# cv-stuttgart/PCFA

Hardware: AMD Instinct MI355X
Metric: attack_steps_per_sec (higher is better)
Workload: dtype f32; 1 GPU; RAFT, 1 synthetic 436x1024 pair per GPU (padded 440x1024), disjoint delta, change_of_variables, delta_bound=0.005, zero target, L-BFGS max_iter=10; weights=random:1234, parallelism=pairs sharded 1/GPU, closure_launch=hipGraph replay

## Files before the change

include/pcfa_hip.h:

```cpp
#ifndef PCFA_HIP_H
#define PCFA_HIP_H

#include <stddef.h>
#include <stdint.h>

#ifdef __cplusplus
extern "C" {
#endif

#define PCFA_OK 0
#define PCFA_ERR_INVALID_ARG (-1)
#define PCFA_ERR_UNSUPPORTED (-2)
#define PCFA_ERR_WORKSPACE (-3)

#if defined(__GNUC__)
#define PCFA_API __attribute__((visibility("default")))
#else
#define PCFA_API
#endif

#define PCFA_MAX_LEVELS 8
#define PCFA_ABI_VERSION 2

#define PCFA_LOSS_AEE 0
// ... 221 lines not shown
PCFA_API int pcfa_leaky_relu_fwd(const float* x, float* y, float slope, long long n, void* stream);
PCFA_API int pcfa_leaky_relu_bwd(const float* out, const float* grad_out, float* grad_x, float slope, long long n,
                        void* stream);
PCFA_API int pcfa_conv3x3_act_fwd_pair(const float* x, const float* packed, const float* bias, float* out, int K, int N,
                              const float* x2, const float* packed2, const float* bias2, float* out2, int K2, int N2,
                              int H, int W, int act, float slope, void* stream);
PCFA_API int pcfa_conv3x3_fused_bwd(const float* g, const float* packed_bwd, const float* mask, const float* addend,
                           float* grad_in, int B, int K, int N, int H, int W, void* stream);
PCFA_API int pcfa_conv3x3_masked_fwd(const float* x, const float* packed, const float* mask, float* out, int B, int K,
                            int N, int H, int W, void* stream);
PCFA_API int pcfa_conv3x3_algo(int B, int K, int N, int H, int W);
PCFA_API size_t pcfa_conv3x3_workspace_bytes(int B, int K, int N, int H, int W);
PCFA_API int pcfa_conv3x3_run(const float* x, const float* packed, const float* bias, const float* mask,
                     const float* addend, float* out, int B, int K, int N, int H, int W, int act, float slope,
                     int mask_channels, void* workspace, size_t workspace_bytes, void* stream);

PCFA_API int pcfa_bias_relu_fwd(const float* x, const float* bias, float* out, long long n, int plane, int channels,
                       void* stream);
PCFA_API int pcfa_relu_bwd(const float* out, const float* grad_out, float* grad_x, long long n, void* stream);
PCFA_API int pcfa_relu_bwd2(const float* out, const float* out2, const float* grad_out, float* grad_x, float* grad_x2,
                   long long n, void* stream);

PCFA_API int pcfa_conv_fewin_fwd(const float* x, const float* w, const float* bias, float* out, int B, int Cin, int N,
                                 int H, int W, int ksize, int relu, void* stream);
PCFA_API long long pcfa_conv_fewin_packed_floats(int Cin, int N, int ksize);
PCFA_API int pcfa_conv_fewin_pack(const float* w, float* packed, int Cin, int N, int ksize, void* stream);
PCFA_API int pcfa_conv_fewin_packed_fwd(const float* x, const float* packed, const float* bias, float* out, int B, int Cin,
                               int N, int H, int W, int ksize, int relu, void* stream);

PCFA_API int pcfa_conv_s2_supported(int Cin, int N, int ksize, int H, int W);
// ... 115 lines not shown
```

pcfa_amd/_hip.py:

```python
import ctypes
import os
from ctypes import c_char_p, c_double, c_float, c_int, c_longlong, c_size_t, c_uint, c_void_p, POINTER

ABI_VERSION = 2
LIB_PATH = os.environ.get("PCFA_HIP_LIB") or os.path.join(os.path.dirname(os.path.abspath(__file__)), "lib",
                                                          "libpcfa_hip.so")

PCFA_LOSS = {"aee": 0, "mse": 1, "cosim": 2}


class HipLibraryError(RuntimeError):
    pass


_P = c_void_p
_S4 = POINTER(c_longlong)

SIGNATURES = {
    "pcfa_abi_version": (c_int, []),
    "pcfa_timing_arm": (c_int, [_P, _P, c_int]),
    "pcfa_null_launch": (c_int, [_P]),
    "pcfa_poison_lds": (c_int, [c_uint, _P]),
    "pcfa_peek_lds": (c_int, [_P, c_int, _P]),
    "pcfa_calib_mfma_f32": (c_longlong, [_P, c_int, c_int, _P]),
# ... 83 lines not shown
                                            c_int, c_int, _P]),
    "pcfa_sepconv5_gru_update_bwd": (c_int, [_P, c_int, c_int, _P, _P, _P, _P, _P, _P, _P, _P, _P, c_int, c_int, c_int,
                                             c_int, _P]),
    "pcfa_convex_upsample_fwd": (c_int, [_P, _P, _P, c_int, c_int, c_int, _P]),
    "pcfa_convex_upsample_workspace_floats": (c_longlong, [c_int, c_int, c_int]),
    "pcfa_convex_upsample_bwd": (c_int, [_P, _P, _P, _P, _P, _P, c_int, c_int, c_int, _P]),
    "pcfa_flow_step": (c_int, [_P, _P, _P, _P, _P, c_longlong, _P]),
    "pcfa_conv3x3_act_fwd_pair": (c_int, [_P, _P, _P, _P, c_int, c_int, _P, _P, _P, _P, c_int, c_int, c_int, c_int, c_int,
                                          c_float, _P]),
    "pcfa_relu_bwd2": (c_int, [_P, _P, _P, _P, _P, c_longlong, _P]),
    "pcfa_conv3x3_fused_bwd": (c_int, [_P, _P, _P, _P, _P, c_int, c_int, c_int, c_int, c_int, _P]),
    "pcfa_conv3x3_masked_fwd": (c_int, [_P, _P, _P, _P, c_int, c_int, c_int, c_int, c_int, _P]),
    "pcfa_conv3x3_algo": (c_int, [c_int] * 5),
    "pcfa_conv3x3_workspace_bytes": (c_size_t, [c_int] * 5),
    "pcfa_conv3x3_run": (c_int, [_P] * 6 + [c_int] * 6 + [c_float, c_int, _P, c_size_t, _P]),
    "pcfa_conv3x3_packed_floats": (c_longlong, [c_int, c_int]),
    "pcfa_conv3x3_pack_weights": (c_int, [_P, _P, _P, c_int, c_int, _P]),
    "pcfa_conv3x3_fwd": (c_int, [_P, _P, _P, _P, c_int, c_int, c_int, c_int, c_int, c_int, _P]),
    "pcfa_conv3x3_act_fwd": (c_int, [_P, _P, _P, _P, c_int, c_int, c_int, c_int, c_int, c_int, c_float, _P]),
    "pcfa_leaky_relu_fwd": (c_int, [_P, _P, c_float, c_longlong, _P]),
    "pcfa_leaky_relu_bwd": (c_int, [_P, _P, _P, c_float, c_longlong, _P]),
    "pcfa_lbfgs_gram_state_bytes": (c_size_t, [c_int]),
    "pcfa_lbfgs_gram_workspace_bytes": (c_size_t, [c_int, c_longlong]),
    "pcfa_lbfgs_gram_reset": (c_int, [_P, c_int, _P]),
    "pcfa_lbfgs_gram_update": (c_int, [_P, _P, _P, c_float, _P, _P, _P, _P, c_int, c_longlong, _P]),
    "pcfa_lbfgs_gram_direction": (c_int, [_P, _P, _P, _P, _P, _P, _P, c_int, c_longlong, _P]),
    "pcfa_lbfgs_workspace_floats": (c_size_t, []),
    "pcfa_lbfgs_pair": (c_int, [_P, _P, _P, c_float, _P, _P, _P, _P, c_int, c_longlong, _P]),
    "pcfa_lbfgs_direction": (c_int, [_P, _P, _P, _P, _P, _P, _P, _P, c_int, c_int, c_int, c_longlong, c_longlong,
                                     _P]),
# ... 96 lines not shown
```

pcfa_amd/config.py:

```python
import dataclasses
import os


def _env_bool(name, default):
    v = os.environ.get(name)
    return default if v is None else v not in ("0", "", "false", "False")


@dataclasses.dataclass(frozen=True)
class Config:
    fused_lookup: bool = True
    overlap_encoders: bool = False
    conv_s2: bool = True
    conv_s2_bwd: bool = True
    fused_downsample: bool = True
    defer_relu: bool = True
    pyramid_bwd_windows: bool = True
    gma_gemm: str = "lib"
    gma_attention: str = "materialised"
    conv1x1: str = "lib"
    corr: str = "all_pairs"
    ondemand_lookup: str = "per_query"
    mfma: str = "f32"
    dilated_as_subgrids: tuple = (2, 4, 8, 16)
    deconv_fewout: bool = True
    defer_leaky: bool = True
    dense_block_fused_masks: bool = True
    warp_bwd_deterministic: bool = True
    pwc_fold_glue: bool = True
    spynet_ops: str = "lib"
    flownet2_ops: str = "lib"
    reuse_pair_graphs: bool = True
    max_cached_shapes: int = 4

    @classmethod
    def from_env(cls):
        return cls(fused_lookup=_env_bool("PCFA_FUSED_LOOKUP", True),
                   overlap_encoders=_env_bool("PCFA_OVERLAP_ENCODERS", False),
                   defer_relu=_env_bool("PCFA_DEFER_RELU", True),
                   gma_gemm=os.environ.get("PCFA_GMA_GEMM", "lib"),
                   gma_attention=os.environ.get("PCFA_GMA_ATTENTION", "materialised"),
                   conv1x1=os.environ.get("PCFA_CONV1X1", "lib"),
                   corr=os.environ.get("PCFA_CORR", "all_pairs"),
                   ondemand_lookup=os.environ.get("PCFA_ONDEMAND_LOOKUP", "per_query"),
                   mfma=os.environ.get("PCFA_MFMA", "f32"),
                   spynet_ops=os.environ.get("PCFA_SPYNET_OPS", "lib"),
                   flownet2_ops=os.environ.get("PCFA_FLOWNET2_OPS", "lib"),
                   max_cached_shapes=int(os.environ.get("PCFA_MAX_CACHED_SHAPES", "4")))

    def __post_init__(self):
        if self.gma_gemm not in ("lib", "hip"):
            raise ValueError("Config.gma_gemm must be 'lib' or 'hip', got %r" % (self.gma_gemm,))
        if self.gma_attention not in ("materialised", "streamed"):
            raise ValueError("Config.gma_attention must be 'materialised' or 'streamed', got %r" % (self.gma_attention,))
        if self.conv1x1 not in ("lib", "hip"):
            raise ValueError("Config.conv1x1 must be 'lib' or 'hip', got %r" % (self.conv1x1,))
        if self.corr not in ("all_pairs", "on_demand"):
            raise ValueError("Config.corr must be 'all_pairs' or 'on_demand', got %r" % (self.corr,))
        if self.ondemand_lookup not in ("per_query", "tiled"):
            raise ValueError("Config.ondemand_lookup must be 'per_query' or 'tiled', got %r" % (self.ondemand_lookup,))
        if self.mfma not in ("f32", "bf16x3"):
            raise ValueError("Config.mfma must be 'f32' or 'bf16x3', got %r" % (self.mfma,))
        if self.spynet_ops not in ("lib", "hip"):
# ... 22 lines not shown
```

pcfa_amd/csrc/conv3x3.hip:

```cpp
#include "common.hpp"
#include "conv3x3_f43.hpp"
#include "conv_tail.hpp"
#include <cstdlib>

namespace {

typedef float f32x16 __attribute__((ext_vector_type(16)));

constexpr int TC = 8;
constexpr int PC = 2 * TC + 2;
constexpr int PCP = 20;
constexpr int KC = 8;
constexpr int CB = 64;

__global__ void conv3x3_pack_kernel(const float* __restrict__ w, float* __restrict__ P, int Cout, int Cin,
                                    int backward, int K, int N, int nchunk, long long total) {
  for (long long e = (long long)blockIdx.x * blockDim.x + threadIdx.x; e < total;
       e += (long long)gridDim.x * blockDim.x) {
    const int pos = (int)(e & 15), lane = (int)((e >> 4) & 63), wv = (int)((e >> 10) & 3);
    const long long blk = e >> 12;
    const int c = (int)(blk % nchunk), nb = (int)(blk / nchunk);
    const int a = pos >> 2, kpi = pos & 3;
    const int i = wv, j = a;
    const int k = 8 * c + 2 * kpi + (lane >> 5), n = 32 * nb + (lane & 31);
// ... 33 lines not shown
  } while (0)
#else
#define C3_STAMP(k) do {} while (0)
#endif

struct Second {
  const float* x;
  const float* U;
  const float* bias;
  float* out;
  int K, N, nb0;
  int mask_n;
  int ksl;
  int cper;
  PcfaXcdMap xcd;
};

template <int ACT, int CBT, int MT, bool KFULL, int NRING, int KS = 1>
__global__ __launch_bounds__(256 * MT * KS) __attribute__((amdgpu_waves_per_eu(KS == 2 ? 2 : (MT == 1 && NRING == 2 && CBT == 32 ? 3 : (CBT == 64 ? 1 : 2))))) void conv3x3_winograd_kernel(
    const float* __restrict__ x, const float* __restrict__ U, const float* __restrict__ bias,
    const float* __restrict__ mask, const float* __restrict__ addend, float* __restrict__ out, int K, int N, int Npad,
    int H, int W, int blocks_x, float slope, Second second) {
  constexpr int NT = 256 * MT;
  constexpr int TR = 4 * MT, TB = TR * TC;
  constexpr int PR = 2 * TR + 2;
  constexpr int RAW = KC * PR * PCP;
  constexpr int RAW_LOADS = (KC * PR * PC + NT - 1) / NT;
  constexpr int MS = TB + 1;
  constexpr int NB = CBT / 32;
  static_assert(KS == 1 || (KS == 2 && MT == 1 && CBT == 32), "split-K rides on the 256-thread tile");
  constexpr int EPI = 16 * 16 * (TB + 1);
  constexpr int RED = KS == 2 ? 4 * 4 * 16 * 64 : 0;
  constexpr int LDS0 = 2 * KS * RAW > EPI ? 2 * KS * RAW : EPI;
  constexpr int LDSF = RED > LDS0 ? RED : LDS0;
  __shared__ __attribute__((aligned(16))) float smem[LDSF];
  const int kgrp = KS == 1 ? 0 : (int)(threadIdx.x >> 8);
  float* sRaw = smem + kgrp * 2 * RAW;

  const int tid = KS == 1 ? (int)threadIdx.x : (int)(threadIdx.x & 255);
  const int lane = tid & 63, wave = (tid >> 6) & 3, mt = tid >> 8;
  const int l31 = lane & 31, lh = lane >> 5;
  int tileblk = blockIdx.x, nby = blockIdx.y;
  if (second.xcd.a != 0 && !pcfa_xcd_item(second.xcd, (int)blockIdx.x, tileblk, nby)) return;
  const int by = tileblk / blocks_x, bx = tileblk - by * blocks_x;
  const int y0 = by * (2 * TR), x0 = bx * (2 * TC);
  if (nby >= second.nb0) {
    nby -= second.nb0;
    x = second.x;
    U = second.U;
    bias = second.bias;
    out = second.out;
    K = second.K;
    N = second.N;
    mask = nullptr;
    addend = nullptr;
  }
  const int mask_n = second.mask_n;
  const int n0 = nby * CBT;
  if (n0 >= N) return;
  const long long plane = (long long)H * W;
  const int ksl = second.ksl, img = blockIdx.z / ksl, slice = blockIdx.z - img * ksl;
  x += (long long)img * K * plane;
  out += ((long long)slice * (gridDim.z / ksl) + img) * N * plane;
  if (mask != nullptr) mask += (long long)img * N * plane;
  if (addend != nullptr) addend += (long long)img * N * plane;

  unsigned praw[RAW_LOADS];
  int rdst[RAW_LOADS];
  int rch[RAW_LOADS];
  bool rok[RAW_LOADS];
#pragma unroll
  for (int i = 0; i < RAW_LOADS; ++i) {
    const int e = tid + NT * i;
    const int ch = e / (PR * PC), rem = e - ch * (PR * PC);
    const int r = rem / PC, c = rem - r * PC;
    const int yy = y0 - 1 + r, xx = x0 - 1 + c;
// ... 201 lines not shown
#pragma unroll
      for (int xi = 0; xi < 16; ++xi) m[xi] = sM[(xi * 16 + cl) * MS + e_tile];
      float t0[4], t1[4];
#pragma unroll
      for (int j = 0; j < 4; ++j) {
        t0[j] = m[j] + m[4 + j] + m[8 + j];
        t1[j] = m[4 + j] - m[8 + j] - m[12 + j];
      }
      const float bv = (bias != nullptr && n < N) ? bias[n] : 0.f;
      const float y00 = t0[0] + t0[1] + t0[2] + bv, y01 = t0[1] - t0[2] - t0[3] + bv;
      const float y10 = t1[0] + t1[1] + t1[2] + bv, y11 = t1[1] - t1[2] - t1[3] + bv;
      if (n < N && oy < H && ox < W && worker) {
        const long long oo = (long long)n * plane + (long long)oy * W + ox;
        const bool mall = mask != nullptr && mask_n == 0, mpre = mask != nullptr && mask_n > 0 && n < mask_n;
        const bool add = addend != nullptr;
        const float4 y = conv_tail<ACT>(make_float4(y00, y01, y10, y11), slope, mall, mpre,
                                        [&] { return make_float4(mk[q][0], mk[q][1], mk[q][2], mk[q][3]); }, add,
                                        [&] { return make_float4(ad[q][0], ad[q][1], ad[q][2], ad[q][3]); });
        float* o = out + oo;
        o[0] = y.x;
        if (ox + 1 < W) o[1] = y.y;
        if (oy + 1 < H) {
          o[W] = y.z;
          if (ox + 1 < W) o[W + 1] = y.w;
        }
      }
    }
    __syncthreads();
  }
}

}

// ... 52 lines not shown
  pcfa_launch(leaky_relu_fwd_kernel, dim3((unsigned)min((n + 255) / 256, 4096LL)), dim3(256), 0, (hipStream_t)stream, x, y,
              slope, n);
  PCFA_LAUNCH_CHECK();
  return PCFA_OK;
}

extern "C" int pcfa_leaky_relu_bwd(const float* out, const float* grad_out, float* grad_x, float slope, long long n,
                                   void* stream) {
  if (!out || !grad_out || !grad_x || n < 1) return PCFA_ERR_INVALID_ARG;
  pcfa_launch(leaky_relu_bwd_kernel, dim3((unsigned)min((n + 255) / 256, 4096LL)), dim3(256), 0, (hipStream_t)stream,
              out, grad_out, grad_x, slope, n);
  PCFA_LAUNCH_CHECK();
  return PCFA_OK;
}

static int conv3x3_launch(const float* x, const float* packed, const float* bias, const float* mask, float* out, int B,
                          int K, int N, int H, int W, int act, float slope, void* stream, const float* x2 = nullptr,
                          const float* packed2 = nullptr, const float* bias2 = nullptr, float* out2 = nullptr,
                          int K2 = 0, int N2 = 0, const float* addend = nullptr, int mask_n = 0, int ksl = 1);

extern "C" int pcfa_conv3x3_fwd(const float* x, const float* packed, const float* bias, float* out, int B, int K,
                                int N, int H, int W, int relu, void* stream) {
  return conv3x3_launch(x, packed, bias, nullptr, out, B, K, N, H, W, relu ? 1 : 0, 0.f, stream);
}

extern "C" int pcfa_conv3x3_act_fwd(const float* x, const float* packed, const float* bias, float* out, int B, int K,
                                    int N, int H, int W, int act, float slope, void* stream) {
  return conv3x3_launch(x, packed, bias, nullptr, out, B, K, N, H, W, act, slope, stream);
}

extern "C" int pcfa_conv3x3_masked_fwd(const float* x, const float* packed, const float* mask, float* out, int B, int K,
                                       int N, int H, int W, void* stream) {
  if (!mask) return PCFA_ERR_INVALID_ARG;
  return conv3x3_launch(x, packed, nullptr, mask, out, B, K, N, H, W, 0, 0.f, stream);
// ... 76 lines not shown
  }
  const int ksl = f23_kslices(B, K, N, H, W);
  if (ksl > 1 && workspace && aligned16(workspace) && aligned16(out) && (!mask || aligned16(mask)) &&
      (!addend || aligned16(addend)) && workspace_bytes >= (size_t)ksl * B * N * H * W * sizeof(float)) {
    float* part = (float*)workspace;
    const int rc = conv3x3_launch(x, packed, nullptr, nullptr, part, B, K, N, H, W, 0, 0.f, stream, nullptr, nullptr,
                                  nullptr, nullptr, 0, 0, nullptr, 0, ksl);
    if (rc != PCFA_OK) return rc;
    return pcfa_f43_finish(part, bias, mask, addend, out, ksl, B, N, H, W, act, slope, mask_channels, (hipStream_t)stream,
                           23);
  }
  return conv3x3_launch(x, packed, bias, mask, out, B, K, N, H, W, act, slope, stream, nullptr, nullptr, nullptr,
                        nullptr, 0, 0, addend, mask_channels);
}

static int conv3x3_launch(const float* x, const float* packed, const float* bias, const float* mask, float* out, int B,
                          int K, int N, int H, int W, int act, float slope, void* stream, const float* x2,
                          const float* packed2, const float* bias2, float* out2, int K2, int N2, const float* addend,
                          int mask_n, int ksl) {
  if (act < 0 || act > 2 || mask_n < 0 || (mask_n > 0 && (act != 0 || !mask))) return PCFA_ERR_INVALID_ARG;
  if (!x || !packed || !out || B < 1 || K < 1 || N < 1 || H < 1 || W < 1 || !aligned16(packed))
    return PCFA_ERR_INVALID_ARG;
  const int Npad = (N + CB - 1) / CB * CB;
  const int blocks_x = pcfa_cdiv(W, 2 * TC), blocks_y = pcfa_cdiv(H, 8);
  const long long gx = (long long)blocks_x * blocks_y;
  if (gx > 0x7fffffffLL || B > 65535 || Npad / CB > 65535 || (long long)K * H * W > 0x7fffffffLL ||
      f23_packed_floats(K, N) > 0x7fffffffLL)
    return PCFA_ERR_UNSUPPORTED;
  dim3 grid((unsigned)gx, Npad / CB, B), block(256);
  hipStream_t s = (hipStream_t)stream;
  int mt = 1;
  if (const char* e = getenv("PCFA_CONV3X3_MT")) mt = atoi(e) == 2 ? 2 : 1;
  if (ksl > 1 || x2 != nullptr) mt = 1;
  if (mt == 2) {
    const int by2 = pcfa_cdiv(H, 16);
    grid.x = (unsigned)(blocks_x * by2);
    block.x = 512;
  }
  grid.y = Npad / 32;
  const int nchunk_all = (K + KC - 1) / KC, cper = (nchunk_all + ksl - 1) / ksl;
  if (ksl > 1) {
    if (x2 != nullptr || bias || mask || addend || act != 0 || (cper * (ksl - 1)) >= nchunk_all) return PCFA_ERR_INVALID_ARG;
    grid.z = (unsigned)(B * ksl);
    if (grid.z > 65535) return PCFA_ERR_UNSUPPORTED;
  }
  Second second{x2, packed2, bias2, out2, K2, N2, (int)grid.y, mask_n, ksl, cper, PcfaXcdMap{0, 0, 0, 0}};
  if (x2 != nullptr) {
    grid.y += (unsigned)((N2 + CB - 1) / CB * CB / 32);
    if (grid.y > 65535) return PCFA_ERR_UNSUPPORTED;
  }
  const long long nwg = (long long)grid.x * grid.y * grid.z;
  static const bool xcd_on = !(getenv("PCFA_XCD_MAP") && atoi(getenv("PCFA_XCD_MAP")) == 0);
  if (xcd_on && mt == 1 && (long long)grid.x * grid.y >= 1024) {
    second.xcd = pcfa_xcd_pick((int)grid.x, (int)grid.y, 4.0 * K * H * W, 4.0 * 16 * K * 32 * grid.y);
    if (second.xcd.a != 0) {
      grid.x = pcfa_xcd_grid(second.xcd);
      grid.y = 1;
    }
  }
#define PCFA_C3_ARGS grid, block, 0, s, x, packed, bias, mask, addend, out, K, N, Npad, H, W, blocks_x, slope, second
#define PCFA_C3_LAUNCH(MT_, KF_, NR_)                                                              \
  do {                                                                                             \
    if (act == 1) pcfa_launch(conv3x3_winograd_kernel<1, 32, MT_, KF_, NR_>, PCFA_C3_ARGS);        \
    else if (act == 2) pcfa_launch(conv3x3_winograd_kernel<2, 32, MT_, KF_, NR_>, PCFA_C3_ARGS);   \
    else pcfa_launch(conv3x3_winograd_kernel<0, 32, MT_, KF_, NR_>, PCFA_C3_ARGS);                 \
  } while (0)
  const bool kfull = K % KC == 0;
  static const int ks_env = getenv("PCFA_CONV3X3_KS") ? atoi(getenv("PCFA_CONV3X3_KS")) : 0;
  if (ksl == 1 && mt == 1 && x2 == nullptr && K % (2 * KC) == 0 && (ks_env ? ks_env == 2 : nwg <= 256)) {
    block.x = 512;
    if (act == 1) pcfa_launch(conv3x3_winograd_kernel<1, 32, 1, true, 2, 2>, PCFA_C3_ARGS);
    else if (act == 2) pcfa_launch(conv3x3_winograd_kernel<2, 32, 1, true, 2, 2>, PCFA_C3_ARGS);
    else pcfa_launch(conv3x3_winograd_kernel<0, 32, 1, true, 2, 2>, PCFA_C3_ARGS);
    PCFA_LAUNCH_CHECK();
    return PCFA_OK;
  }
  int deep = 0;
  if (const char* e = getenv("PCFA_CONV3X3_RING")) deep = atoi(e) == 3;
  if (mt == 2) {
    if (kfull) PCFA_C3_LAUNCH(2, true, 2); else PCFA_C3_LAUNCH(2, false, 2);
  } else if (deep) {
    if (kfull) PCFA_C3_LAUNCH(1, true, 3); else PCFA_C3_LAUNCH(1, false, 3);
// ... 9 lines not shown
```

pcfa_amd/nets/gma.py:

```python
import torch
import torch.nn as nn

from .. import ops
from ..config import cfg
from .raft import (BasicEncoder, BasicMotionEncoder, FlowHead, LookupRef, SepConvGRU, _mask_head, convex_upsample,
                   _f32, coords_grid, mask_logits, mfma_kw)


class RelPosEmb(nn.Module):
    def __init__(self, max_pos_size, dim_head):
        super().__init__()
        self.rel_height = nn.Embedding(2 * max_pos_size - 1, dim_head)
        self.rel_width = nn.Embedding(2 * max_pos_size - 1, dim_head)
        deltas = torch.arange(max_pos_size).view(1, -1) - torch.arange(max_pos_size).view(-1, 1)
        self.register_buffer('rel_ind', deltas + max_pos_size - 1)

    def forward(self, q):
        b, heads, h, w, c = q.shape
        height_emb = self.rel_height(self.rel_ind[:h, :h].reshape(-1)).view(h, h, 1, c)
        width_emb = self.rel_width(self.rel_ind[:w, :w].reshape(-1)).view(w, 1, w, c)
        height_score = torch.einsum('bhxyd,xuvd->bhxyuv', q, height_emb)
        width_score = torch.einsum('bhxyd,yuvd->bhxyuv', q, width_emb)
        return height_score + width_score

# ... 137 lines not shown
            args.dropout = 0
        self.fnet = BasicEncoder(output_dim=256, norm_fn='instance', dropout=args.dropout)
        self.cnet = BasicEncoder(output_dim=hdim + cdim, norm_fn='batch', dropout=args.dropout)
        self.update_block = GMAUpdateBlock(args, hidden_dim=hdim)
        self.att = Attention(args=args, dim=cdim, heads=args.num_heads, max_pos_size=160, dim_head=cdim)

    def freeze_bn(self):
        for m in self.modules():
            if isinstance(m, nn.BatchNorm2d):
                m.eval()

    def forward(self, image1, image2, iters=12, flow_init=None, upsample=True, test_mode=False):
        images12, image1 = ops.get().pm1_pair(image1, image2)
        hdim, cdim = self.hidden_dim, self.context_dim

        fmap1, fmap2 = self.fnet(images12, split=image1.shape[0])
        if cfg(self).corr == "on_demand":
            corr_fn = ops.get().OnDemandCorrBlock(_f32(fmap1), _f32(fmap2), num_levels=4, radius=self.args.corr_radius,
                                                  lookup=cfg(self).ondemand_lookup)
        else:
            corr_fn = ops.get().CorrBlock(_f32(fmap1), _f32(fmap2), num_levels=4, radius=self.args.corr_radius,
                                          bwd_windows=cfg(self).pyramid_bwd_windows, **mfma_kw(cfg(self)))

        net, inp = torch.split(self.cnet(image1), [hdim, cdim], dim=1)
        net, inp = torch.tanh(net), torch.relu(inp)
        attention = self.att(inp)

        N, _, H, W = image1.shape
        coords0 = coords_grid(N, H // 8, W // 8, image1.device, _f32(image1).dtype)
        coords1 = coords_grid(N, H // 8, W // 8, image1.device, _f32(image1).dtype)
        if flow_init is not None:
            coords1 = coords1 + flow_init

        gru = self.update_block.gru
        gru_ctx = gru.per_iteration(gru.precompute(inp), iters) if gru.frozen() else None
        flow_predictions = []
        flow_up = None
        o = ops.get()
        attn_grad = o.AttnGradShare(cfg(self).gma_gemm, cfg(self).mfma) if hasattr(o, "AttnGradShare") else _SharedAttnGrad()
# ... 17 lines not shown
```

pcfa_amd/nets/raft.py:

```python

import torch
import torch.nn as nn
import torch.nn.functional as F

from .. import ops
from ..config import cfg


def _norm(kind, planes):
    if kind == 'batch':
        return nn.BatchNorm2d(planes)
    if kind == 'instance':
        return nn.InstanceNorm2d(planes)
    if kind == 'group':
        return nn.GroupNorm(num_groups=planes // 8, num_channels=planes)
    if kind == 'none':
        return nn.Sequential()
    raise ValueError("unknown norm_fn %r" % kind)


def _fold_batchnorm(conv, bn, cache, tag):
    tensors = (conv.weight, conv.bias, bn.weight, bn.bias, bn.running_mean, bn.running_var)
    key = tuple((t.data_ptr(), t._version) for t in tensors if t is not None) + (conv.weight.device,)
    hit = cache.get(tag)
# ... 83 lines not shown
        if not (cfg(self).fused_downsample and _all_frozen(self) and conv1.stride == (2, 2) and convd.stride == (2, 2)
                and convd.kernel_size == (1, 1) and convd.padding == (0, 0) and _is_stride2(conv1, x, cfg(self))
                and o.conv_s2_ds_supported(x, conv1.weight, convd.weight)):
            return None
        if all(isinstance(n, nn.BatchNorm2d) and not n.training and n.track_running_stats for n in (n1, nd)):
            w1, b1 = _fold_batchnorm(conv1, n1, self._fold_cache, "1")
            wd, bd = _fold_batchnorm(convd, nd, self._fold_cache, "d")
            if not o.conv_s2_ds_supported(x, w1, wd):
                return None
            return o.conv_s2_ds(x, w1, wd, b1, bd, relu=True)
        if all(isinstance(n, nn.InstanceNorm2d) and not n.affine and not n.track_running_stats for n in (n1, nd)):
            y, xd = o.conv_s2_ds(x, conv1.weight, convd.weight)
            return o.instance_norm_relu(y, n1.eps, True), o.instance_norm_relu(xd, nd.eps, False)
        return None

    def forward(self, x):
        pair = self._entry_pair(x) if self.downsample is not None else None
        if pair is not None:
            y, xd = pair
            y = _conv_norm(self.conv2, self.norm2, y, True, self._fold_cache, "2")
            return ops.get().add_relu(xd, y)
        if self.downsample is None and _all_frozen(self) and _can_skip(self.conv1, self.norm1):
            y, x = _conv_norm(self.conv1, self.norm1, x, True, self._fold_cache, "1", skip=True,
                              grad_premasked=cfg(self).defer_relu and isinstance(self.norm1, nn.BatchNorm2d) and isinstance(self.norm2, nn.BatchNorm2d)
                              and _can_skip(self.conv2, self.norm2))
        else:
            y = _conv_norm(self.conv1, self.norm1, x, True, self._fold_cache, "1")
        chain = (cfg(self).defer_relu and _all_frozen(self) and isinstance(self.norm2, nn.BatchNorm2d) and _can_skip(self.conv2, self.norm2)
                 and _can_skip(self.conv1, self.norm1) and self.downsample is None)
        y = _conv_norm(self.conv2, self.norm2, y, True, self._fold_cache, "2", grad_premasked=chain, mask_input_grad=chain)
# ... 40 lines not shown
            x = torch.cat(x, dim=0)
        x = _conv_norm(self.conv1, self.norm1, x, True, self._fold_cache, "1")
        x = self.layer3(self.layer2(self.layer1(x)))
        x = _conv1x1(self.conv2, x, cfg(self))
        if self.training and self.dropout is not None:
            x = self.dropout(x)
        if pair:
            x = torch.split(x, [n, n], dim=0)
        return x


def _all_frozen(module):
    return not any(p.requires_grad for p in module.parameters())


def _conv_nobias(conv, x):
    return conv._conv_forward(x, conv.weight, None)


def _is_plain3x3(conv, min_out=16):
    return (conv.kernel_size == (3, 3) and conv.stride == (1, 1) and conv.padding == (1, 1) and conv.dilation == (1, 1)
            and conv.groups == 1 and conv.padding_mode == "zeros" and conv.out_channels >= min_out)


def _is_plain1x1(conv):
    return (conv.kernel_size == (1, 1) and conv.stride == (1, 1) and conv.padding == (0, 0) and conv.dilation == (1, 1)
            and conv.groups == 1)


def mfma_kw(config):
# ... 218 lines not shown
        self.args.setdefault("dropout", 0)
        self.fnet = BasicEncoder(output_dim=256, norm_fn='instance', dropout=self.args["dropout"])
        self.cnet = BasicEncoder(output_dim=hdim + cdim, norm_fn='batch', dropout=self.args["dropout"])
        self.update_block = BasicUpdateBlock(4, 4, hidden_dim=hdim)

    def freeze_bn(self):
        for m in self.modules():
            if isinstance(m, nn.BatchNorm2d):
                m.eval()

    def forward(self, image1, image2, iters=12, flow_init=None, upsample=True, test_mode=False):
        images12, image1 = ops.get().pm1_pair(image1, image2)
        hdim, cdim = self.hidden_dim, self.context_dim

        side = None
        if cfg(self).overlap_encoders and image1.is_cuda and hasattr(ops.get(), "side_stream"):
            main = torch.cuda.current_stream()
            side = ops.get().side_stream(image1.device)
            side.wait_stream(main)
            with torch.cuda.stream(side):
                cnet_out = self.cnet(image1)
        fmap1, fmap2 = self.fnet(images12, split=image1.shape[0])
        if cfg(self).corr == "on_demand":
            corr_fn = ops.get().OnDemandCorrBlock(_f32(fmap1), _f32(fmap2), num_levels=self.args["corr_levels"],
                                                  radius=self.args["corr_radius"], lookup=cfg(self).ondemand_lookup)
        else:
            corr_fn = ops.get().CorrBlock(_f32(fmap1), _f32(fmap2), num_levels=self.args["corr_levels"],
                                          radius=self.args["corr_radius"], bwd_windows=cfg(self).pyramid_bwd_windows,
                                          **mfma_kw(cfg(self)))
        if side is not None:
            main.wait_stream(side)
        else:
            cnet_out = self.cnet(image1)

        net, inp = torch.split(cnet_out, [hdim, cdim], dim=1)
        net, inp = torch.tanh(net), torch.relu(inp)

        N, _, H, W = image1.shape
        coords0 = coords_grid(N, H // 8, W // 8, image1.device, _f32(image1).dtype)
        coords1 = coords_grid(N, H // 8, W // 8, image1.device, _f32(image1).dtype)
        if flow_init is not None:
            coords1 = coords1 + flow_init

        gru = self.update_block.gru
        gru_ctx = gru.per_iteration(gru.precompute(inp), iters) if gru.frozen() else None
        flow_predictions = []
        flow_up = None
# ... 16 lines not shown
```

pcfa_amd/ops/conv.py:

```python
import ctypes
import os

import torch

from .. import _hip
from . import core
from .core import _call, _dev, _ptr, _ptr_off, cached_pack, current_lane


FEWIN_SHAPES = {(2, 7), (1, 7), (2, 5), (2, 3)}
_FEWIN_PACKED = os.environ.get("PCFA_FEWIN_PACKED", "1") != "0"


def _pack_cin_n_k(w, pack, packed_floats):
    N, Cin, k, _ = w.shape
    w = w.contiguous()
    packed = torch.empty(int(getattr(_hip.load(), packed_floats)(Cin, N, k)), device=w.device, dtype=torch.float32)
    _call(pack, _ptr(w), _ptr(packed), Cin, N, k)
    return packed


def _fewin_packed(weight):
    return cached_pack("fewin", (weight,),
                       lambda w: _pack_cin_n_k(w, "pcfa_conv_fewin_pack", "pcfa_conv_fewin_packed_floats"))
# ... 439 lines not shown
        B, K, N, H, W = ctx.dims
        if g is None:
            return (None if g_skip is None else g_skip), None, None, None, None, None, None, None
        g = g.contiguous()
        if ctx.act and not ctx.grad_premasked:
            g = _act_bwd(ctx.saved_tensors[0], g, ctx.act, ctx.slope)
        gin = torch.empty((B, K, H, W), device=g.device, dtype=torch.float32)
        if g_skip is not None or ctx.mask_input_grad:
            xin = ctx.saved_tensors[-1] if ctx.mask_input_grad else None
            _conv3x3_run(g.device, _ptr(g), ctx.bwd, None, _ptr(xin),
                         _ptr(None if g_skip is None else g_skip.contiguous()), _ptr(gin), B, N, K, H, W,
                         slope=ctx.input_slope if ctx.mask_input_grad else 0.)
        else:
            _conv3x3_run(g.device, _ptr(g), ctx.bwd, None, None, None, _ptr(gin), B, N, K, H, W)
        return gin, None, None, None, None, None, None, None


_PAIR_LAUNCH = os.environ.get("PCFA_CONV3X3_PAIR", "1") != "0"


class _Conv3x3Cat(torch.autograd.Function):

    @staticmethod
    def forward(ctx, n_conv, flags, *args):
        xs, ws, bs = args[0:3 * n_conv:3], args[1:3 * n_conv:3], args[2:3 * n_conv:3]
        tails = args[3 * n_conv:]
        ctx.grad_premasked, ctx.mask_input_grads = bool(flags & 1), bool(flags & 2)
        _dev(*xs, *ws, *tails)
        xs = [x.contiguous() for x in xs]
        B, _, H, W = xs[0].shape
# ... 156 lines not shown
```

pcfa_amd/ops/core.py:

```python
import contextlib
import ctypes
import threading
import weakref

import torch

from .. import _hip

_lane_state = threading.local()
_STREAM_LANE = {}


def current_lane():
    if _STREAM_LANE and torch.cuda.is_available():
        k = _STREAM_LANE.get(torch.cuda.current_stream().cuda_stream)
        if k is not None:
            return k
    return getattr(_lane_state, "k", 0)


@contextlib.contextmanager
def lane(k):
    prev = getattr(_lane_state, "k", 0)
    _lane_state.k = int(k)
# ... 160 lines not shown
        _note_work("conv3x3_winograd", direct, direct / 2.25)


def _sepconv5_work(B, Ca, Cb, Cout, H, W, vertical):
    direct = 2.0 * 5 * (Ca + Cb) * Cout * B * H * W
    if _hip.load().pcfa_sepconv5_uses_winograd(B, Ca, Cb, Cout, H, W, int(vertical)):
        _note_work("sepconv5_winograd", direct, direct * 0.6)
    else:
        _note_work("sepconv5_direct", direct, direct)


_WORK_TABLE = {
    "pcfa_conv3x3_run": lambda a: _conv3x3_work(a[6], a[7], a[8], a[9], a[10]),
    "pcfa_conv3x3_act_fwd_pair": lambda a: (_conv3x3_work(1, a[4], a[5], a[12], a[13]),
                                            _conv3x3_work(1, a[10], a[11], a[12], a[13])),
    "pcfa_sepconv5_fwd": lambda a: _sepconv5_work(a[6], a[1], a[3], a[7], a[8], a[9], a[10]),
    "pcfa_sepconv5_fwd_split": lambda a: _sepconv5_work(a[10], a[1], a[3], a[11], a[12], a[13], a[14]),
    "pcfa_sepconv5_fwd_split_masked": lambda a: _sepconv5_work(a[12], a[1], a[3], a[13], a[14], a[15], a[16]),
    "pcfa_sepconv5_gru_gates_fwd": lambda a: _sepconv5_work(a[9], a[1], a[3], 2 * a[1], a[10], a[11], a[12]),
    "pcfa_sepconv5_gru_update_fwd": lambda a: _sepconv5_work(a[10], a[1], a[3], a[1], a[11], a[12], a[13]),
    "pcfa_sepconv5_gru_gates_bwd": lambda a: _sepconv5_work(a[13], a[1], 0, a[1] + a[2], a[14], a[15], a[16]),
    "pcfa_sepconv5_gru_update_bwd": lambda a: _sepconv5_work(a[12], 2 * a[1], 0, a[1] + a[2], a[13], a[14], a[15]),
    "pcfa_instnorm_fwd": lambda a: _note_work("instnorm_fwd", 2.0 * a[4] * a[5] * 4, 0.0),
    "pcfa_instnorm_bwd": lambda a: _note_work("instnorm_bwd", 3.0 * a[5] * a[6] * 4, 0.0),
    "pcfa_conv3x3_fewout_fwd": lambda a: _note_work("conv3x3_fewout_fwd", 4.0 * a[5] * (a[6] + a[7]) * a[8] * a[9], 0.0),
    "pcfa_conv3x3_fewout_bwd": lambda a: _note_work("conv3x3_fewout_bwd", 4.0 * a[4] * (a[5] + a[6]) * a[7] * a[8], 0.0),
    "pcfa_relu_bwd": lambda a: _note_work("relu_bwd", 12.0 * a[3], 0.0),
    "pcfa_relu_bwd2": lambda a: _note_work("relu_bwd2", 20.0 * a[5], 0.0),
    "pcfa_add_relu_fwd": lambda a: _note_work("add_relu_fwd", 12.0 * a[3], 0.0),
    "pcfa_conv_fewin_packed_fwd": lambda a: _note_work("conv_fewin_fwd", *(2 * [2.0 * a[5] * a[9] * a[9] * a[6] * a[4] * a[7] * a[8]])),
# ... 60 lines not shown
```

Baseline: 7.570 attack_steps/s.

## Fuse fnet and cnet encoder 3x3 convolutions into single paired-image launches

Adds a paired-image conv3x3 Winograd launch in which extra grid.z slices process a second network's input with its own weights, bias, mask, addend and activation. The RAFT and GMA forward passes now walk the frozen feature and context encoders in lockstep, issuing one launch per matching conv for both forward and backward. This is on by default whenever encoder overlap is off. The aim is fewer kernel launches and better GPU fill for small-batch encoder convs, at the cost of a runtime activation branch inside the kernel and a longer Python gating path.

```diff
diff --git a/include/pcfa_hip.h b/include/pcfa_hip.h
--- a/include/pcfa_hip.h
+++ b/include/pcfa_hip.h
@@ -259,6 +259,12 @@
 PCFA_API int pcfa_conv3x3_run(const float* x, const float* packed, const float* bias, const float* mask,
                      const float* addend, float* out, int B, int K, int N, int H, int W, int act, float slope,
                      int mask_channels, void* workspace, size_t workspace_bytes, void* stream);
+PCFA_API int pcfa_conv3x3_pair_images_supported(int B, int K, int N, int B2, int K2, int N2, int H, int W);
+PCFA_API int pcfa_conv3x3_run_pair_images(const float* x, const float* packed, const float* bias, const float* mask,
+                                 const float* addend, float* out, int B, int K, int N, int act, float slope,
+                                 int mask_channels, const float* x2, const float* packed2, const float* bias2,
+                                 const float* mask2, const float* addend2, float* out2, int B2, int K2, int N2, int act2,
+                                 float slope2, int mask_channels2, int H, int W, int H2, int W2, void* stream);
 
 PCFA_API int pcfa_bias_relu_fwd(const float* x, const float* bias, float* out, long long n, int plane, int channels,
                        void* stream);
diff --git a/pcfa_amd/_hip.py b/pcfa_amd/_hip.py
--- a/pcfa_amd/_hip.py
+++ b/pcfa_amd/_hip.py
@@ -121,6 +121,8 @@
     "pcfa_conv3x3_algo": (c_int, [c_int] * 5),
     "pcfa_conv3x3_workspace_bytes": (c_size_t, [c_int] * 5),
     "pcfa_conv3x3_run": (c_int, [_P] * 6 + [c_int] * 6 + [c_float, c_int, _P, c_size_t, _P]),
+    "pcfa_conv3x3_pair_images_supported": (c_int, [c_int] * 8),
+    "pcfa_conv3x3_run_pair_images": (c_int, 2 * ([_P] * 6 + [c_int] * 4 + [c_float, c_int]) + [c_int] * 4 + [_P]),
     "pcfa_conv3x3_packed_floats": (c_longlong, [c_int, c_int]),
     "pcfa_conv3x3_pack_weights": (c_int, [_P, _P, _P, c_int, c_int, _P]),
     "pcfa_conv3x3_fwd": (c_int, [_P, _P, _P, _P, c_int, c_int, c_int, c_int, c_int, c_int, _P]),
diff --git a/pcfa_amd/config.py b/pcfa_amd/config.py
--- a/pcfa_amd/config.py
+++ b/pcfa_amd/config.py
@@ -1,5 +1,6 @@
 import dataclasses
 import os
+import typing
 
 
 def _env_bool(name, default):
@@ -11,6 +12,7 @@
 class Config:
     fused_lookup: bool = True
     overlap_encoders: bool = False
+    pair_encoders: typing.Optional[bool] = None
     conv_s2: bool = True
     conv_s2_bwd: bool = True
     fused_downsample: bool = True
@@ -37,6 +39,7 @@
     def from_env(cls):
         return cls(fused_lookup=_env_bool("PCFA_FUSED_LOOKUP", True),
                    overlap_encoders=_env_bool("PCFA_OVERLAP_ENCODERS", False),
+                   pair_encoders=_env_bool("PCFA_PAIR_ENCODERS", None),
                    defer_relu=_env_bool("PCFA_DEFER_RELU", True),
                    gma_gemm=os.environ.get("PCFA_GMA_GEMM", "lib"),
                    gma_attention=os.environ.get("PCFA_GMA_ATTENTION", "materialised"),
@@ -47,6 +50,9 @@
                    spynet_ops=os.environ.get("PCFA_SPYNET_OPS", "lib"),
                    flownet2_ops=os.environ.get("PCFA_FLOWNET2_OPS", "lib"),
                    max_cached_shapes=int(os.environ.get("PCFA_MAX_CACHED_SHAPES", "4")))
+
+    def pairs_encoders(self):
+        return (not self.overlap_encoders) if self.pair_encoders is None else bool(self.pair_encoders)
 
     def __post_init__(self):
         if self.gma_gemm not in ("lib", "hip"):
diff --git a/pcfa_amd/csrc/conv3x3.hip b/pcfa_amd/csrc/conv3x3.hip
--- a/pcfa_amd/csrc/conv3x3.hip
+++ b/pcfa_amd/csrc/conv3x3.hip
@@ -2,6 +2,7 @@
 #include "conv3x3_f43.hpp"
 #include "conv_tail.hpp"
 #include <cstdlib>
+#include <type_traits>
 
 namespace {
 
@@ -71,6 +72,11 @@
   int ksl;
   int cper;
   PcfaXcdMap xcd;
+  int b0;
+  const float* mask2;
+  const float* addend2;
+  int mask_n2, act1, act2;
+  float slope2;
 };
 
 template <int ACT, int CBT, int MT, bool KFULL, int NRING, int KS = 1>
@@ -101,8 +107,11 @@
   if (second.xcd.a != 0 && !pcfa_xcd_item(second.xcd, (int)blockIdx.x, tileblk, nby)) return;
   const int by = tileblk / blocks_x, bx = tileblk - by * blocks_x;
   const int y0 = by * (2 * TR), x0 = bx * (2 * TC);
-  if (nby >= second.nb0) {
-    nby -= second.nb0;
+  const int ksl = second.ksl, slice = blockIdx.z % ksl;
+  int img = blockIdx.z / ksl, mask_n = second.mask_n;
+  int act = ACT == 3 ? second.act1 : ACT;
+  const bool p2img = img >= second.b0;
+  if (nby >= second.nb0 || p2img) {
     x = second.x;
     U = second.U;
     bias = second.bias;
@@ -111,12 +120,20 @@
     N = second.N;
     mask = nullptr;
     addend = nullptr;
-  }
-  const int mask_n = second.mask_n;
+    if (p2img) {
+      img -= second.b0;
+      mask = second.mask2;
+      addend = second.addend2;
+      mask_n = second.mask_n2;
+      act = second.act2;
+      slope = second.slope2;
+    } else {
+      nby -= second.nb0;
+    }
+  }
   const int n0 = nby * CBT;
   if (n0 >= N) return;
   const long long plane = (long long)H * W;
-  const int ksl = second.ksl, img = blockIdx.z / ksl, slice = blockIdx.z - img * ksl;
   x += (long long)img * K * plane;
   out += ((long long)slice * (gridDim.z / ksl) + img) * N * plane;
   if (mask != nullptr) mask += (long long)img * N * plane;
@@ -348,9 +365,16 @@
         const long long oo = (long long)n * plane + (long long)oy * W + ox;
         const bool mall = mask != nullptr && mask_n == 0, mpre = mask != nullptr && mask_n > 0 && n < mask_n;
         const bool add = addend != nullptr;
-        const float4 y = conv_tail<ACT>(make_float4(y00, y01, y10, y11), slope, mall, mpre,
-                                        [&] { return make_float4(mk[q][0], mk[q][1], mk[q][2], mk[q][3]); }, add,
-                                        [&] { return make_float4(ad[q][0], ad[q][1], ad[q][2], ad[q][3]); });
+        auto tail = [&](auto a) {
+          return conv_tail<decltype(a)::value>(make_float4(y00, y01, y10, y11), slope, mall, mpre,
+                                               [&] { return make_float4(mk[q][0], mk[q][1], mk[q][2], mk[q][3]); }, add,
+                                               [&] { return make_float4(ad[q][0], ad[q][1], ad[q][2], ad[q][3]); });
+        };
+        float4 y;
+        if constexpr (ACT != 3) y = tail(std::integral_constant<int, ACT>{});
+        else
+          y = act == 1 ? tail(std::integral_constant<int, 1>{}) : act == 2 ? tail(std::integral_constant<int, 2>{})
+                                                                         : tail(std::integral_constant<int, 0>{});
         float* o = out + oo;
         o[0] = y.x;
         if (ox + 1 < W) o[1] = y.y;
@@ -433,10 +457,23 @@
   return PCFA_OK;
 }
 
+struct ImagePair {
+  const float* x;
+  const float* packed;
+  const float* bias;
+  const float* mask;
+  const float* addend;
+  float* out;
+  int B, K, N, act;
+  float slope;
+  int mask_n;
+};
+
 static int conv3x3_launch(const float* x, const float* packed, const float* bias, const float* mask, float* out, int B,
                           int K, int N, int H, int W, int act, float slope, void* stream, const float* x2 = nullptr,
                           const float* packed2 = nullptr, const float* bias2 = nullptr, float* out2 = nullptr,
-                          int K2 = 0, int N2 = 0, const float* addend = nullptr, int mask_n = 0, int ksl = 1);
+                          int K2 = 0, int N2 = 0, const float* addend = nullptr, int mask_n = 0, int ksl = 1,
+                          const struct ImagePair* ip = nullptr);
 
 extern "C" int pcfa_conv3x3_fwd(const float* x, const float* packed, const float* bias, float* out, int B, int K,
                                 int N, int H, int W, int relu, void* stream) {
@@ -543,10 +580,38 @@
                         nullptr, 0, 0, addend, mask_channels);
 }
 
+static bool run_args_ok(const void* x, const void* packed, const void* mask, const void* out, int B, int K, int N, int act,
+                        int mask_channels) {
+  return x && packed && out && B >= 1 && K >= 1 && N >= 1 && act >= 0 && act <= 2 && mask_channels >= 0 &&
+         mask_channels <= N && !(mask_channels > 0 && (!mask || act != 0)) && !(mask && act == 2);
+}
+
+extern "C" int pcfa_conv3x3_pair_images_supported(int B, int K, int N, int B2, int K2, int N2, int H, int W) {
+  if (B < 1 || K < 1 || N < 1 || B2 < 1 || K2 < 1 || N2 < 1 || H < 1 || W < 1) return 0;
+  if ((K % KC == 0) != (K2 % KC == 0)) return 0;
+  if (use_f43(B, K, N, H, W) || use_f43(B2, K2, N2, H, W)) return 0;
+  return f23_kslices(B, K, N, H, W) == 1 && f23_kslices(B2, K2, N2, H, W) == 1;
+}
+
+extern "C" int pcfa_conv3x3_run_pair_images(const float* x, const float* packed, const float* bias, const float* mask,
+                                            const float* addend, float* out, int B, int K, int N, int act, float slope,
+                                            int mask_channels, const float* x2, const float* packed2, const float* bias2,
+                                            const float* mask2, const float* addend2, float* out2, int B2, int K2, int N2,
+                                            int act2, float slope2, int mask_channels2, int H, int W, int H2, int W2,
+                                            void* stream) {
+  if (H < 1 || W < 1 || H2 < 1 || W2 < 1 || !run_args_ok(x, packed, mask, out, B, K, N, act, mask_channels) ||
+      !run_args_ok(x2, packed2, mask2, out2, B2, K2, N2, act2, mask_channels2) || !aligned16(packed2))
+    return PCFA_ERR_INVALID_ARG;
+  if (H2 != H || W2 != W || !pcfa_conv3x3_pair_images_supported(B, K, N, B2, K2, N2, H, W)) return PCFA_ERR_UNSUPPORTED;
+  const ImagePair ip{x2, packed2, bias2, mask2, addend2, out2, B2, K2, N2, act2, slope2, mask_channels2};
+  return conv3x3_launch(x, packed, bias, mask, out, B, K, N, H, W, act, slope, stream, nullptr, nullptr, nullptr, nullptr,
+                        0, 0, addend, mask_channels, 1, &ip);
+}
+
 static int conv3x3_launch(const float* x, const float* packed, const float* bias, const float* mask, float* out, int B,
                           int K, int N, int H, int W, int act, float slope, void* stream, const float* x2,
                           const float* packed2, const float* bias2, float* out2, int K2, int N2, const float* addend,
-                          int mask_n, int ksl) {
+                          int mask_n, int ksl, const ImagePair* ip) {
   if (act < 0 || act > 2 || mask_n < 0 || (mask_n > 0 && (act != 0 || !mask))) return PCFA_ERR_INVALID_ARG;
   if (!x || !packed || !out || B < 1 || K < 1 || N < 1 || H < 1 || W < 1 || !aligned16(packed))
     return PCFA_ERR_INVALID_ARG;
@@ -560,7 +625,7 @@
   hipStream_t s = (hipStream_t)stream;
   int mt = 1;
   if (const char* e = getenv("PCFA_CONV3X3_MT")) mt = atoi(e) == 2 ? 2 : 1;
-  if (ksl > 1 || x2 != nullptr) mt = 1;
+  if (ksl > 1 || x2 != nullptr || ip != nullptr) mt = 1;
   if (mt == 2) {
     const int by2 = pcfa_cdiv(H, 16);
     grid.x = (unsigned)(blocks_x * by2);
@@ -573,7 +638,17 @@
     grid.z = (unsigned)(B * ksl);
     if (grid.z > 65535) return PCFA_ERR_UNSUPPORTED;
   }
-  Second second{x2, packed2, bias2, out2, K2, N2, (int)grid.y, mask_n, ksl, cper, PcfaXcdMap{0, 0, 0, 0}};
+  Second second{x2, packed2, bias2, out2, K2, N2, (int)grid.y, mask_n, ksl, cper, PcfaXcdMap{0, 0, 0, 0},
+                0x7fffffff, nullptr, nullptr, 0, act, 0, 0.f};
+  if (ip != nullptr) {
+    if (x2 != nullptr || ksl > 1 || (long long)B + ip->B > 65535 || (long long)ip->K * H * W > 0x7fffffffLL ||
+        f23_packed_floats(ip->K, ip->N) > 0x7fffffffLL)
+      return PCFA_ERR_UNSUPPORTED;
+    grid.y = max(grid.y, (unsigned)((ip->N + CB - 1) / CB * CB / 32));
+    grid.z = (unsigned)(B + ip->B);
+    second = Second{ip->x, ip->packed, ip->bias, ip->out, ip->K, ip->N, (int)grid.y, mask_n, 1, cper,
+                    PcfaXcdMap{0, 0, 0, 0}, B, ip->mask, ip->addend, ip->mask_n, act, ip->act, ip->slope};
+  }
   if (x2 != nullptr) {
     grid.y += (unsigned)((N2 + CB - 1) / CB * CB / 32);
     if (grid.y > 65535) return PCFA_ERR_UNSUPPORTED;
@@ -595,6 +670,12 @@
     else pcfa_launch(conv3x3_winograd_kernel<0, 32, MT_, KF_, NR_>, PCFA_C3_ARGS);                 \
   } while (0)
   const bool kfull = K % KC == 0;
+  if (ip != nullptr) {
+    if (kfull) pcfa_launch(conv3x3_winograd_kernel<3, 32, 1, true, 2>, PCFA_C3_ARGS);
+    else pcfa_launch(conv3x3_winograd_kernel<3, 32, 1, false, 2>, PCFA_C3_ARGS);
+    PCFA_LAUNCH_CHECK();
+    return PCFA_OK;
+  }
   static const int ks_env = getenv("PCFA_CONV3X3_KS") ? atoi(getenv("PCFA_CONV3X3_KS")) : 0;
   if (ksl == 1 && mt == 1 && x2 == nullptr && K % (2 * KC) == 0 && (ks_env ? ks_env == 2 : nwg <= 256)) {
     block.x = 512;
diff --git a/pcfa_amd/nets/gma.py b/pcfa_amd/nets/gma.py
--- a/pcfa_amd/nets/gma.py
+++ b/pcfa_amd/nets/gma.py
@@ -4,7 +4,7 @@
 from .. import ops
 from ..config import cfg
 from .raft import (BasicEncoder, BasicMotionEncoder, FlowHead, LookupRef, SepConvGRU, _mask_head, convex_upsample,
-                   _f32, coords_grid, mask_logits, mfma_kw)
+                   _f32, coords_grid, mask_logits, mfma_kw, paired_encoders)
 
 
 class RelPosEmb(nn.Module):
@@ -175,7 +175,11 @@
         images12, image1 = ops.get().pm1_pair(image1, image2)
         hdim, cdim = self.hidden_dim, self.context_dim
 
-        fmap1, fmap2 = self.fnet(images12, split=image1.shape[0])
+        paired = paired_encoders(self.fnet, self.cnet, images12, image1)
+        if paired is not None:
+            fmap1, fmap2, cnet_out = paired
+        else:
+            fmap1, fmap2 = self.fnet(images12, split=image1.shape[0])
         if cfg(self).corr == "on_demand":
             corr_fn = ops.get().OnDemandCorrBlock(_f32(fmap1), _f32(fmap2), num_levels=4, radius=self.args.corr_radius,
                                                   lookup=cfg(self).ondemand_lookup)
@@ -183,7 +187,7 @@
             corr_fn = ops.get().CorrBlock(_f32(fmap1), _f32(fmap2), num_levels=4, radius=self.args.corr_radius,
                                           bwd_windows=cfg(self).pyramid_bwd_windows, **mfma_kw(cfg(self)))
 
-        net, inp = torch.split(self.cnet(image1), [hdim, cdim], dim=1)
+        net, inp = torch.split(cnet_out if paired is not None else self.cnet(image1), [hdim, cdim], dim=1)
         net, inp = torch.tanh(net), torch.relu(inp)
         attention = self.att(inp)
 
diff --git a/pcfa_amd/nets/raft.py b/pcfa_amd/nets/raft.py
--- a/pcfa_amd/nets/raft.py
+++ b/pcfa_amd/nets/raft.py
@@ -121,6 +121,13 @@
             return o.instance_norm_relu(y, n1.eps, True), o.instance_norm_relu(xd, nd.eps, False)
         return None
 
+    def _entry(self, x):
+        pair = self._entry_pair(x)
+        if pair is not None:
+            return pair
+        return (_conv_norm(self.conv1, self.norm1, x, True, self._fold_cache, "1"),
+                _conv_norm(self.downsample[0], self.downsample[1], x, False, self._fold_cache, "d"))
+
     def forward(self, x):
         pair = self._entry_pair(x) if self.downsample is not None else None
         if pair is not None:
@@ -191,6 +198,67 @@
     return not any(p.requires_grad for p in module.parameters())
 
 
+
+def _instance(norm):
+    return isinstance(norm, nn.InstanceNorm2d) and not norm.affine and not norm.track_running_stats
+
+
+def _can_pair_encoders(fnet, cnet, x):
+    if not (cfg(fnet).pairs_encoders() and x.is_cuda and hasattr(ops.get(), "conv3x3_pair")):
+        return False
+    if not (_all_frozen(fnet) and _all_frozen(cnet)):
+        return False
+    if any(e.training and e.dropout is not None for e in (fnet, cnet)):
+        return False
+    if not (_instance(fnet.norm1) and isinstance(cnet.norm1, nn.BatchNorm2d)):
+        return False
+    for lf, lc in zip((fnet.layer1, fnet.layer2, fnet.layer3), (cnet.layer1, cnet.layer2, cnet.layer3)):
+        if len(lf) != len(lc):
+            return False
+        for bf, bc in zip(lf, lc):
+            if (bf.downsample is None) != (bc.downsample is None):
+                return False
+            convs = [("conv2", "norm2")] + ([("conv1", "norm1")] if bf.downsample is None else [])
+            for cname, nname in convs:
+                cf, cc, nf, nc = getattr(bf, cname), getattr(bc, cname), getattr(bf, nname), getattr(bc, nname)
+                if not (_can_skip(cf, nf) and _can_skip(cc, nc) and _instance(nf) and isinstance(nc, nn.BatchNorm2d)
+                        and cf.weight.shape == cc.weight.shape):
+                    return False
+    return True
+
+
+def _block_pair(bf, bc, xf, xc):
+    o = ops.get()
+    if bf.downsample is not None:
+        (yf, rf), (yc, rc) = bf._entry(xf), bc._entry(xc)
+        chain = False
+    else:
+        chain = cfg(bc).defer_relu
+        w1, b1 = _fold_batchnorm(bc.conv1, bc.norm1, bc._fold_cache, "1")
+        (yf, rf), (yc, rc) = o.conv3x3_pair(dict(x=xf, weight=bf.conv1.weight, skip=True),
+                                            dict(x=xc, weight=w1, bias=b1, relu=True, skip=True, grad_premasked=chain))
+        yf = o.instance_norm_relu(yf, bf.norm1.eps, True)
+    w2, b2 = _fold_batchnorm(bc.conv2, bc.norm2, bc._fold_cache, "2")
+    yf, yc = o.conv3x3_pair(dict(x=yf, weight=bf.conv2.weight),
+                            dict(x=yc, weight=w2, bias=b2, relu=True, grad_premasked=chain, mask_input_grad=chain))
+    yf = o.instance_norm_relu(yf, bf.norm2.eps, True)
+    return o.add_relu(rf, yf), o.add_relu(rc, yc, b_is_relu=chain)
+
+
+def paired_encoders(fnet, cnet, images12, image1):
+    if not _can_pair_encoders(fnet, cnet, images12):
+        return None
+    xf = _conv_norm(fnet.conv1, fnet.norm1, images12, True, fnet._fold_cache, "1")
+    xc = _conv_norm(cnet.conv1, cnet.norm1, image1, True, cnet._fold_cache, "1")
+    for lf, lc in zip((fnet.layer1, fnet.layer2, fnet.layer3), (cnet.layer1, cnet.layer2, cnet.layer3)):
+        for bf, bc in zip(lf, lc):
+            xf, xc = _block_pair(bf, bc, xf, xc)
+    xf, xc = _conv1x1(fnet.conv2, xf, cfg(fnet)), _conv1x1(cnet.conv2, xc, cfg(cnet))
+    n = image1.shape[0]
+    fmap1, fmap2 = torch.split(xf, [n, n], dim=0)
+    return fmap1, fmap2, xc
+
+
 def _conv_nobias(conv, x):
     return conv._conv_forward(x, conv.weight, None)
 
@@ -439,13 +507,17 @@
         hdim, cdim = self.hidden_dim, self.context_dim
 
         side = None
-        if cfg(self).overlap_encoders and image1.is_cuda and hasattr(ops.get(), "side_stream"):
+        paired = paired_encoders(self.fnet, self.cnet, images12, image1)
+        if paired is not None:
+            fmap1, fmap2, cnet_out = paired
+        elif cfg(self).overlap_encoders and image1.is_cuda and hasattr(ops.get(), "side_stream"):
             main = torch.cuda.current_stream()
             side = ops.get().side_stream(image1.device)
             side.wait_stream(main)
             with torch.cuda.stream(side):
                 cnet_out = self.cnet(image1)
-        fmap1, fmap2 = self.fnet(images12, split=image1.shape[0])
+        if paired is None:
+            fmap1, fmap2 = self.fnet(images12, split=image1.shape[0])
         if cfg(self).corr == "on_demand":
             corr_fn = ops.get().OnDemandCorrBlock(_f32(fmap1), _f32(fmap2), num_levels=self.args["corr_levels"],
                                                   radius=self.args["corr_radius"], lookup=cfg(self).ondemand_lookup)
@@ -455,7 +527,7 @@
                                           **mfma_kw(cfg(self)))
         if side is not None:
             main.wait_stream(side)
-        else:
+        elif paired is None:
             cnet_out = self.cnet(image1)
 
         net, inp = torch.split(cnet_out, [hdim, cdim], dim=1)
diff --git a/pcfa_amd/ops/conv.py b/pcfa_amd/ops/conv.py
--- a/pcfa_amd/ops/conv.py
+++ b/pcfa_amd/ops/conv.py
@@ -477,6 +477,95 @@
         else:
             _conv3x3_run(g.device, _ptr(g), ctx.bwd, None, None, None, _ptr(gin), B, N, K, H, W)
         return gin, None, None, None, None, None, None, None
+
+
+def _conv3x3_run_pair(device, p1, p2, hw1, hw2):
+    (B, K, N), (B2, K2, N2) = p1[6:9], p2[6:9]
+    if hw1 == hw2 and _hip.load().pcfa_conv3x3_pair_images_supported(B, K, N, B2, K2, N2, hw1[0], hw1[1]):
+        args = []
+        for p in (p1, p2):
+            args += [p[0], _ptr(p[1]), p[2], p[3], p[4], p[5], p[6], p[7], p[8], int(p[9]), float(p[10]), int(p[11])]
+        _call("pcfa_conv3x3_run_pair_images", *args, hw1[0], hw1[1], hw2[0], hw2[1])
+        return
+    for p, (H, W) in ((p1, hw1), (p2, hw2)):
+        _conv3x3_run(device, p[0], p[1], p[2], p[3], p[4], p[5], p[6], p[7], p[8], H, W, p[9], p[10], p[11])
+
+
+class _Conv3x3Pair(torch.autograd.Function):
+
+    @staticmethod
+    def forward(ctx, xa, wa, ba, opta, xb, wb, bb, optb):
+        _dev(xa, wa, ba, xb, wb, bb)
+        ctx.set_materialize_grads(False)
+        ctx.opts = (tuple(bool(o) for o in opta), tuple(bool(o) for o in optb))
+        runs, results, saved, hold, ctx.bwd, ctx.dims, ctx.slots = [], [], [], [], [], [], []
+        for x, w, b, (relu, skip, premasked, mask_in) in ((xa, wa, ba, ctx.opts[0]), (xb, wb, bb, ctx.opts[1])):
+            if w.dim() != 4 or tuple(w.shape[2:]) != (3, 3) or w.dtype != torch.float32:
+                raise ValueError("conv3x3_pair expects float32 3x3 Conv2d weights, got %s" % (tuple(w.shape),))
+            if x.dim() != 4 or w.shape[1] != x.shape[1]:
+                raise ValueError("conv3x3_pair: input %s does not match weight %s" % (tuple(x.shape), tuple(w.shape)))
+            if premasked and not relu:
+                raise ValueError("conv3x3_pair: grad_premasked needs relu=True")
+            x = x.contiguous()
+            hold.append(x)
+            B, K, H, W = x.shape
+            N = w.shape[0]
+            fwd, bwd = _conv3x3_packed(w)
+            out = torch.empty((B, N, H, W), device=x.device, dtype=torch.float32)
+            runs.append(((_ptr(x), fwd, _ptr(b), None, None, _ptr(out), B, K, N, int(relu), 0., 0), (H, W)))
+            ctx.bwd.append(bwd)
+            ctx.dims.append((B, K, N, H, W))
+            slot = [None, None]
+            if relu and not premasked:
+                slot[0] = len(saved)
+                saved.append(out)
+            if mask_in:
+                slot[1] = len(saved)
+                saved.append(x)
+            ctx.slots.append(slot)
+            results += [out, x.view_as(x)] if skip else [out]
+        _conv3x3_run_pair(xa.device, runs[0][0], runs[1][0], runs[0][1], runs[1][1])
+        ctx.save_for_backward(*saved)
+        return tuple(results)
+
+    @staticmethod
+    def backward(ctx, *grads):
+        if any(ctx.needs_input_grad[i] for i in (1, 2, 5, 6)):
+            raise RuntimeError("conv3x3_pair is the frozen-weight path: no weight / bias gradient")
+        grads = list(grads)
+        gins, runs, keep = [None, None], [], []
+        for i, (relu, skip, premasked, mask_in) in enumerate(ctx.opts):
+            g = grads.pop(0)
+            g_skip = grads.pop(0) if skip else None
+            B, K, N, H, W = ctx.dims[i]
+            if g is None:
+                gins[i] = g_skip
+                continue
+            g = g.contiguous()
+            if relu and not premasked:
+                g = _act_bwd(ctx.saved_tensors[ctx.slots[i][0]], g, 1)
+            xin = ctx.saved_tensors[ctx.slots[i][1]] if mask_in else None
+            g_skip = None if g_skip is None else g_skip.contiguous()
+            gins[i] = torch.empty((B, K, H, W), device=g.device, dtype=torch.float32)
+            keep += [g, g_skip]
+            runs.append(((_ptr(g), ctx.bwd[i], None, _ptr(xin), _ptr(g_skip), _ptr(gins[i]), B, N, K, 0, 0., 0), (H, W)))
+        if len(runs) == 2:
+            _conv3x3_run_pair(keep[0].device, runs[0][0], runs[1][0], runs[0][1], runs[1][1])
+        for p, (H, W) in runs if len(runs) == 1 else ():
+            _conv3x3_run(keep[0].device, p[0], p[1], p[2], p[3], p[4], p[5], p[6], p[7], p[8], H, W)
+        return gins[0], None, None, None, gins[1], None, None, None
+
+
+def conv3x3_pair(a, b):
+    flat, skips = [], []
+    for p in (a, b):
+        skips.append(bool(p.get("skip", False)))
+        flat += [p["x"], p["weight"], p.get("bias"), (p.get("relu", False), skips[-1], p.get("grad_premasked", False),
+                                                      p.get("mask_input_grad", False))]
+    res = list(_Conv3x3Pair.apply(*flat))
+    ra = (res.pop(0), res.pop(0)) if skips[0] else res.pop(0)
+    rb = (res.pop(0), res.pop(0)) if skips[1] else res.pop(0)
+    return ra, rb
 
 
 _PAIR_LAUNCH = os.environ.get("PCFA_CONV3X3_PAIR", "1") != "0"
diff --git a/pcfa_amd/ops/core.py b/pcfa_amd/ops/core.py
--- a/pcfa_amd/ops/core.py
+++ b/pcfa_amd/ops/core.py
@@ -198,6 +198,8 @@
     "pcfa_conv3x3_run": lambda a: _conv3x3_work(a[6], a[7], a[8], a[9], a[10]),
     "pcfa_conv3x3_act_fwd_pair": lambda a: (_conv3x3_work(1, a[4], a[5], a[12], a[13]),
                                             _conv3x3_work(1, a[10], a[11], a[12], a[13])),
+    "pcfa_conv3x3_run_pair_images": lambda a: (_conv3x3_work(a[6], a[7], a[8], a[24], a[25]),
+                                               _conv3x3_work(a[18], a[19], a[20], a[24], a[25])),
     "pcfa_sepconv5_fwd": lambda a: _sepconv5_work(a[6], a[1], a[3], a[7], a[8], a[9], a[10]),
     "pcfa_sepconv5_fwd_split": lambda a: _sepconv5_work(a[10], a[1], a[3], a[11], a[12], a[13], a[14]),
     "pcfa_sepconv5_fwd_split_masked": lambda a: _sepconv5_work(a[12], a[1], a[3], a[13], a[14], a[15], a[16]),
```

New measurement: 7.637 attack_steps/s, median of 6. About the same (+0.9%).
